# johndpope/SPEAK-hack

Hardware: NVIDIA B200
Metric: irfd_train_pairs_per_sec_256 (higher is better)
Workload: dtype bf16

## Files before the change

### speak_hack_b200/csrc/conv_gemm.cu

```cuda
#include <stdlib.h>

#include "host_util.h"
#include "ptx.cuh"

namespace irfd {

enum { EPI_PLAIN = 0, EPI_STATS = 1, EPI_STYLE = 2, EPI_AFFINE = 3, EPI_BNBWD = 4, EPI_BNBWD_RES = 5 };

struct ConvGemmArgs {
  int M_total, N_total;
  int num_m_tiles, num_n_tiles;
  int taps, kw, pad, cin_chunks;
  int H, W, HW, B;
  const float* bias;
  const float* nw;
  const float* noise;
  const float* sp1;
  const float* s1;
  float* stat_sum;
  float* stat_sq;
  const __nv_bfloat16* res;
  __nv_bfloat16* y_lo;
  int wg_tiles;
  int a_mod_tiles;
  int relu;
  const __nv_bfloat16* bn_z;
  const __nv_bfloat16* bn_g2;
  const uint8_t* bn_bits;
  const float* bn_mean;
  const float* bn_rstd;
  const float* bn_gamma[4];
  const float* bn_beta[4];
  int sg_tiles;
  int warp_epi;
};

constexpr int kNumThreads = 320;
constexpr int kEpiThreads = 256;
constexpr int kMiscBytes = 12 * 1024;
constexpr int kStgBytes = 16384;
constexpr int kSmemLimit = 232448;

template <int BLOCK_N, int MODE>
struct GemmCfg {
  static constexpr int A_BYTES = 128 * 128;
  static constexpr int B_BYTES = BLOCK_N * 128;
  static constexpr int STAGE_BYTES = A_BYTES + B_BYTES;
  static constexpr int NUM_OUT = (MODE == EPI_STYLE) ? 2 : 1;
  static constexpr int STG_TOTAL = 4 * kStgBytes;
  static constexpr int RAW_STAGES = (kSmemLimit - 1024 - STG_TOTAL - kMiscBytes) / STAGE_BYTES;
  static constexpr int STAGES = RAW_STAGES > 8 ? 8 : RAW_STAGES;
  static constexpr int SMEM_BYTES = 1024 + STAGES * STAGE_BYTES + STG_TOTAL + kMiscBytes;
  static constexpr uint32_t TMEM_COLS = (2 * BLOCK_N <= 128) ? 128 : (2 * BLOCK_N <= 256 ? 256 : 512);
};

template <int BLOCK_N, int MODE, int NBUF>
__device__ __forceinline__ void epilogue_acc(const ConvGemmArgs& p, const CUtensorMap* map_out,
                                             const CUtensorMap* map_out2, uint32_t tmem_base, uint32_t acc_col,
                                             int m0, int n_tile, uint64_t* release_bar, uint8_t* stg_base, float* vec,
                                             uint32_t& chunk_counter) {
  const int warp = threadIdx.x >> 5;
  const int lane = threadIdx.x & 31;
  const int e = warp - 2;
  const int q = warp & 3;
  const int half = e >> 2;
  const int etid = threadIdx.x - 64;
  const int r = q * 32 + lane;
  float* vb = vec;
  float* vnw = vec + 256;
  float* vsp1 = vec + 512;
  float* vs1 = vec + 1024;
  const int m_tile = m0 >> 7;
  const int ng0 = n_tile * BLOCK_N;
  const int pg0 = (m_tile / p.wg_tiles) * p.N_total + ng0;
  float noise_r = 0.f;
  int img_local = 0;
  if constexpr (MODE == EPI_STYLE) {
    const int nimg = p.HW < 128 ? 128 / p.HW : 1;
    const int b0 = m0 / p.HW;
    for (int i = etid; i < BLOCK_N; i += kEpiThreads) {
      vb[i] = p.bias[ng0 + i];
      vnw[i] = p.nw[ng0 + i];
    }
    for (int i = etid; i < nimg * BLOCK_N; i += kEpiThreads) {
      const int img = i / BLOCK_N, c = i - img * BLOCK_N;
      int bb = b0 + img;
      if (bb >= p.B) bb = p.B - 1;
      vsp1[img * 256 + c] = p.sp1[(size_t)bb * p.N_total + ng0 + c];
      vs1[img * 256 + c] = p.s1[(size_t)bb * p.N_total + ng0 + c];
    }
    named_bar_sync(1, kEpiThreads);
    if (m0 + r < p.M_total) noise_r = p.noise[m0 + r];
    img_local = p.HW < 128 ? r / p.HW : 0;
  } else if constexpr (MODE == EPI_PLAIN) {
    if (p.bias != nullptr) {
      for (int i = etid; i < BLOCK_N; i += kEpiThreads) vb[i] = p.bias[pg0 + i];
      named_bar_sync(1, kEpiThreads);
    }
  } else if constexpr (MODE == EPI_AFFINE) {
    for (int i = etid; i < BLOCK_N; i += kEpiThreads) {
      vb[i] = p.bias[pg0 + i];
      vnw[i] = p.nw[pg0 + i];
// ... 150 lines not shown
          tma_store_commit();
        }
      }
      if (etid < 128) {
        const int ch = etid & 63, which = etid >> 6;
        float acc = 0.f;
#pragma unroll
        for (int gg = 0; gg < 8; ++gg) acc += red[(gg * 64 + ch) * 2 + which];
        p.stat_sum[((size_t)m_tile * 2 + which) * p.N_total + ng0 + chunk * 64 + ch] = acc;
      }
      continue;
    }
    if (warp == 2) {
      __syncwarp();
      if (elect_one_sync()) {
        tma_store_2d(map_out, stg0, ng0 + chunk * 64, m0);
        if constexpr (MODE == EPI_STYLE) tma_store_2d(map_out2, stg1, ng0 + chunk * 64, m0);
        tma_store_commit();
      }
    }
    if constexpr (MODE == EPI_STATS) {
      const int pr = etid & 31;
      const int g = etid >> 5;
      float s0 = 0.f, s1 = 0.f, q0 = 0.f, q1 = 0.f;
#pragma unroll
      for (int i = 0; i < 16; ++i) {
        const int row = g * 16 + i;
        const int phys = (pr >> 2) ^ (row & 7);
        const uint32_t w = *reinterpret_cast<const uint32_t*>(stg0 + row * 128 + phys * 16 + (pr & 3) * 4);
        const float2 f = unpack_bf16x2(w);
        s0 += f.x;
        q0 += f.x * f.x;
        s1 += f.y;
        q1 += f.y * f.y;
      }
      float* red = vec;
      red[(g * 64 + 2 * pr) * 2 + 0] = s0;
      red[(g * 64 + 2 * pr) * 2 + 1] = q0;
      red[(g * 64 + 2 * pr + 1) * 2 + 0] = s1;
      red[(g * 64 + 2 * pr + 1) * 2 + 1] = q1;
      named_bar_sync(1, kEpiThreads);
      if (etid < 128) {
        const int ch = etid & 63, which = etid >> 6;
        float acc = 0.f;
#pragma unroll
        for (int gg = 0; gg < 8; ++gg) acc += red[(gg * 64 + ch) * 2 + which];
        float* dst = which ? p.stat_sq : p.stat_sum;
        dst[(size_t)m_tile * p.N_total + ng0 + chunk * 64 + ch] = acc;
      }
    }
  }
}

constexpr int kSlabBytes = 4096;

template <int BLOCK_N, int MODE>
__device__ __forceinline__ void epilogue_tile_warp(const ConvGemmArgs& p, const CUtensorMap* map_slab, uint32_t tmem_base,
                                                   uint32_t acc_col, int m0, int n_tile, uint64_t* release_bar,
                                                   uint8_t* stg_base, float* vec, uint32_t& chunk_counter,
                                                   uint32_t& my_slabs, bool release_at_leader = false) {
  static_assert(MODE != EPI_STYLE, "STYLE keeps the two-output epilogue");
  auto release = [&]() {
    if (release_at_leader) mbar_arrive_cluster(release_bar, 0);
    else mbar_arrive(release_bar);
  };
  constexpr int CHUNKS = BLOCK_N / 64;
  constexpr bool kSums = MODE == EPI_STATS || MODE == EPI_BNBWD || MODE == EPI_BNBWD_RES;
  const int warp = threadIdx.x >> 5;
  const int lane = threadIdx.x & 31;
  const int e = warp - 2;
  const int q = warp & 3;
  const int h = e >> 2;
  const int m_tile = m0 >> 7;
  const int ng0 = n_tile * BLOCK_N;
  const int pg0 = (m_tile / p.wg_tiles) * p.N_total + ng0;
  const int row = m0 + q * 32 + lane;
  uint8_t* slabs = stg_base + e * 2 * kSlabBytes;
  float* wvec = vec + e * 128;
  const int first = (h - (int)chunk_counter) & 1;
  const int last_mine = first < CHUNKS ? first + 2 * ((CHUNKS - 1 - first) / 2) : -1;
  if (last_mine < 0) {
    __syncwarp();
    if (lane == 0) release();
  }
#pragma unroll 1
  for (int chunk = first; chunk < CHUNKS; chunk += 2) {
    const int cg0 = ng0 + chunk * 64;
    uint32_t zw[32], gw[32];
    uint8_t bw[32];
    if constexpr (MODE == EPI_BNBWD || MODE == EPI_BNBWD_RES) {
      const size_t cell0 = (size_t)(m0 + q * 32) * p.N_total + cg0 + 2 * lane;
#pragma unroll
      for (int i = 0; i < 32; ++i) {
        zw[i] = __ldg(reinterpret_cast<const uint32_t*>(p.bn_z + cell0 + (size_t)i * p.N_total));
        if constexpr (MODE == EPI_BNBWD_RES) {
          gw[i] = __ldg(reinterpret_cast<const uint32_t*>(p.bn_g2 + cell0 + (size_t)i * p.N_total));
          bw[i] = __ldg(p.bn_bits + ((cell0 + (size_t)i * p.N_total) >> 3));
        }
      }
    }
    if constexpr (MODE == EPI_AFFINE || MODE == EPI_PLAIN) {
      if (MODE == EPI_AFFINE || p.bias != nullptr) {
        __syncwarp();
        wvec[lane] = MODE == EPI_AFFINE ? p.nw[pg0 + chunk * 64 + lane] : 0.f;
        wvec[lane + 32] = MODE == EPI_AFFINE ? p.nw[pg0 + chunk * 64 + 32 + lane] : 0.f;
        wvec[64 + lane] = p.bias[pg0 + chunk * 64 + lane];
        wvec[96 + lane] = p.bias[pg0 + chunk * 64 + 32 + lane];
        __syncwarp();
      }
    }
    uint32_t va[32], vb[32];
    const uint32_t taddr = tmem_base + (uint32_t(q * 32) << 16) + acc_col + chunk * 64;
    tmem_ld32(taddr, va);
    tmem_ld32(taddr + 32, vb);
    tmem_ld_wait();
    if (chunk == last_mine) {
      tc_fence_before();
      __syncwarp();
      if (lane == 0) release();
    }
    uint8_t* slab = slabs + (my_slabs & 1) * kSlabBytes;
    if (lane == 0) tma_store_wait_read<1>();
    __syncwarp();
#pragma unroll
    for (int j = 0; j < 8; ++j) {
      float o[8];
#pragma unroll
      for (int t = 0; t < 8; ++t) {
        const int c = j * 8 + t;
        const float acc = __uint_as_float(c < 32 ? va[c & 31] : vb[c & 31]);
        if constexpr (MODE == EPI_AFFINE) o[t] = acc * wvec[c] + wvec[64 + c];
        else if constexpr (MODE == EPI_PLAIN) o[t] = p.bias != nullptr ? acc + wvec[64 + c] : acc;
        else o[t] = acc;
      }
      if constexpr (MODE == EPI_AFFINE) {
        if (p.res != nullptr && row < p.M_total) {
          const uint4 u = *reinterpret_cast<const uint4*>(p.res + (size_t)row * p.N_total + cg0 + j * 8);
          const float2 a0 = unpack_bf16x2(u.x), a1 = unpack_bf16x2(u.y), a2 = unpack_bf16x2(u.z), a3 = unpack_bf16x2(u.w);
          o[0] += a0.x; o[1] += a0.y; o[2] += a1.x; o[3] += a1.y;
          o[4] += a2.x; o[5] += a2.y; o[6] += a3.x; o[7] += a3.y;
        }
#pragma unroll
        for (int t = 0; t < 8; ++t)
          o[t] = p.relu == 1 ? fmaxf(o[t], 0.f) : (p.relu == 2 ? (o[t] > 0.f ? o[t] : 0.2f * o[t]) : o[t]);
      }
      uint4 pk;
      pk.x = pack_bf16x2(o[0], o[1]);
      pk.y = pack_bf16x2(o[2], o[3]);
      pk.z = pack_bf16x2(o[4], o[5]);
      pk.w = pack_bf16x2(o[6], o[7]);
      *reinterpret_cast<uint4*>(slab + lane * 128 + ((j ^ (lane & 7)) << 4)) = pk;
    }
    if constexpr (kSums) {
      __syncwarp();
      float s0 = 0.f, s1 = 0.f, q0 = 0.f, q1 = 0.f;
      if constexpr (MODE == EPI_STATS) {
#pragma unroll
        for (int i = 0; i < 32; ++i) {
          const uint32_t w = *reinterpret_cast<const uint32_t*>(slab + i * 128 + (((lane >> 2) ^ (i & 7)) << 4) + (lane & 3) * 4);
          const float2 f = unpack_bf16x2(w);
          s0 += f.x;
          q0 += f.x * f.x;
          s1 += f.y;
          q1 += f.y * f.y;
        }
      } else {
        const int cc = cg0 + 2 * lane;
        const size_t so = (size_t)(m_tile / p.sg_tiles) * p.N_total + cc;
        const float2 mm = __ldg(reinterpret_cast<const float2*>(p.bn_mean + so));
        const float2 rs = __ldg(reinterpret_cast<const float2*>(p.bn_rstd + so));
        float2 ga = make_float2(0.f, 0.f), be = make_float2(0.f, 0.f);
        if constexpr (MODE == EPI_BNBWD) {
          const int grp = m_tile / p.wg_tiles;
          const float* gam =
              grp == 0 ? p.bn_gamma[0] : (grp == 1 ? p.bn_gamma[1] : (grp == 2 ? p.bn_gamma[2] : p.bn_gamma[3]));
          const float* bet = grp == 0 ? p.bn_beta[0] : (grp == 1 ? p.bn_beta[1] : (grp == 2 ? p.bn_beta[2] : p.bn_beta[3]));
          ga = __ldg(reinterpret_cast<const float2*>(gam + cc));
          be = __ldg(reinterpret_cast<const float2*>(bet + cc));
        }
        const int bit0 = (2 * lane) & 7;
#pragma unroll
        for (int i = 0; i < 32; ++i) {
          uint32_t* cell = reinterpret_cast<uint32_t*>(slab + i * 128 + (((lane >> 2) ^ (i & 7)) << 4) + (lane & 3) * 4);
          float2 f = unpack_bf16x2(*cell);
          const float2 z = unpack_bf16x2(zw[i]);
          const float x0 = (z.x - mm.x) * rs.x, x1 = (z.y - mm.y) * rs.y;
          if constexpr (MODE == EPI_BNBWD) {
            f.x = (ga.x * x0 + be.x) > 0.f ? f.x : 0.f;
            f.y = (ga.y * x1 + be.y) > 0.f ? f.y : 0.f;
          } else {
            const float2 g2 = unpack_bf16x2(gw[i]);
            f.x = ((bw[i] >> bit0) & 1) ? f.x + g2.x : 0.f;
            f.y = ((bw[i] >> (bit0 + 1)) & 1) ? f.y + g2.y : 0.f;
          }
          *cell = pack_bf16x2(f.x, f.y);
          s0 += f.x;
          q0 += f.x * x0;
          s1 += f.y;
          q1 += f.y * x1;
        }
      }
      float* red = vec + ((((my_slabs & 1) * 2 + h) * 4 + q) * 64) * 2;
      *reinterpret_cast<float4*>(red + 4 * lane) = make_float4(s0, q0, s1, q1);
    }
    fence_proxy_async_smem();
    __syncwarp();
    if (lane == 0) {
      tma_store_2d(map_slab, slab, cg0, m0 + q * 32);
      tma_store_commit();
    }
    if constexpr (kSums) {
      named_bar_sync(1 + h, 128);
      if (q == 0) {
        const float* r0 = vec + ((((my_slabs & 1) * 2 + h) * 4) * 64) * 2 + 4 * lane;
        float4 t = *reinterpret_cast<const float4*>(r0);
#pragma unroll
        for (int k = 1; k < 4; ++k) {
          const float4 u = *reinterpret_cast<const float4*>(r0 + k * 128);
          t.x += u.x;
          t.y += u.y;
          t.z += u.z;
          t.w += u.w;
        }
        if constexpr (MODE == EPI_STATS) {
          const size_t d = (size_t)m_tile * p.N_total + cg0 + 2 * lane;
          *reinterpret_cast<float2*>(p.stat_sum + d) = make_float2(t.x, t.z);
          *reinterpret_cast<float2*>(p.stat_sq + d) = make_float2(t.y, t.w);
        } else {
          const size_t d = (size_t)m_tile * 2 * p.N_total + cg0 + 2 * lane;
          *reinterpret_cast<float2*>(p.stat_sum + d) = make_float2(t.x, t.z);
          *reinterpret_cast<float2*>(p.stat_sum + d + p.N_total) = make_float2(t.y, t.w);
        }
      }
    }
    ++my_slabs;
  }
  chunk_counter += CHUNKS;
}

template <int BLOCK_N, int MODE, int CL = 1, bool MMA2 = false>
__global__ void __launch_bounds__(kNumThreads, 1)
conv_gemm_kernel(const __grid_constant__ CUtensorMap map_a, const __grid_constant__ CUtensorMap map_b,
                 const __grid_constant__ CUtensorMap map_out, const __grid_constant__ CUtensorMap map_out2,
                 const ConvGemmArgs p) {
  using Cfg = GemmCfg<BLOCK_N, MODE>;
  constexpr int STAGES = Cfg::STAGES;
  static_assert(STAGES >= 2, "pipeline too shallow");
  static_assert(!MMA2 || (CL == 2 && MODE != EPI_STYLE), "the 2-SM MMA needs a CTA pair and the per-warp epilogue");

  extern __shared__ uint8_t smem_raw[];
  uint8_t* smem = reinterpret_cast<uint8_t*>((reinterpret_cast<uintptr_t>(smem_raw) + 1023) & ~uintptr_t(1023));
  uint8_t* stg_base = smem + STAGES * Cfg::STAGE_BYTES;
  uint8_t* misc = stg_base + Cfg::STG_TOTAL;
  float* vec = reinterpret_cast<float*>(misc);
  uint64_t* full_bar = reinterpret_cast<uint64_t*>(misc + 8192);
  uint64_t* empty_bar = full_bar + STAGES;
  uint64_t* tmem_full = empty_bar + STAGES;
  uint64_t* tmem_empty = tmem_full + 2;
  uint32_t* tmem_ptr = reinterpret_cast<uint32_t*>(tmem_empty + 2);

  const int warp = threadIdx.x >> 5;
  const int lane = threadIdx.x & 31;
  const int crank = CL > 1 ? (int)cluster_ctarank() : 0;
  const int unit0 = blockIdx.x / CL, unit_step = gridDim.x / CL;
  const int total_units = (p.num_m_tiles / CL) * p.num_n_tiles;
  const int num_kb = p.taps * p.cin_chunks;
  constexpr uint16_t kClusterMask = (1u << CL) - 1;

  if (threadIdx.x == 0) {
    for (int i = 0; i < STAGES; ++i) {
      mbar_init(&full_bar[i], 1);
      mbar_init(&empty_bar[i], MMA2 ? 1 : CL);
    }
    for (int i = 0; i < 2; ++i) {
      mbar_init(&tmem_full[i], 1);
      mbar_init(&tmem_empty[i], MMA2 ? 16 : 8);
    }
    fence_mbar_init();
  }
  __syncwarp();
  if (warp == 0) {
    if (MMA2) tmem_alloc_2sm<Cfg::TMEM_COLS>(tmem_ptr);
    else tmem_alloc<Cfg::TMEM_COLS>(tmem_ptr);
  }
  tc_fence_before();
  __syncthreads();
  if (CL > 1) cluster_sync_all();
  tc_fence_after();
  const uint32_t tmem_base = *tmem_ptr;

  if (warp == 0) {
    {
      if (lane == 0) {
        tma_prefetch_desc(&map_a);
        tma_prefetch_desc(&map_b);
      }
      __syncwarp();
      int stage = 0;
      uint32_t phase = 0;
      for (int unit = unit0; unit < total_units; unit += unit_step) {
        const int m_tile = (unit / p.num_n_tiles) * CL + crank;
        const int n_tile = unit % p.num_n_tiles;
        const int m0 = (p.a_mod_tiles > 0 ? m_tile % p.a_mod_tiles : m_tile) * 128;
        const int w0 = m0 % p.W;
        const int h0 = (m0 / p.W) % p.H;
        const int n0 = m0 / (p.W * p.H);
        const int b_row = (m_tile / p.wg_tiles) * p.N_total + n_tile * BLOCK_N;
        for (int tap = 0; tap < p.taps; ++tap) {
          const int dh = tap / p.kw - p.pad;
          const int dw = tap % p.kw - p.pad;
          for (int ch = 0; ch < p.cin_chunks; ++ch) {
            mbar_wait(&empty_bar[stage], phase ^ 1);
            uint8_t* sa = smem + stage * Cfg::STAGE_BYTES;
            if (MMA2) {
              if (elect_one_sync()) {
                if (crank == 0) mbar_expect_tx(&full_bar[stage], 2 * (Cfg::A_BYTES + Cfg::B_BYTES / 2));
                tma_load_4d_2sm(sa, &map_a, &full_bar[stage], ch * 64, w0 + dw, h0 + dh, n0);
                tma_load_2d_2sm(sa + Cfg::A_BYTES, &map_b, &full_bar[stage], (tap * p.cin_chunks + ch) * 64,
                                b_row + crank * (BLOCK_N / 2));
              }
            } else if (elect_one_sync()) {
              mbar_expect_tx(&full_bar[stage], Cfg::STAGE_BYTES);
              tma_load_4d(sa, &map_a, &full_bar[stage], ch * 64, w0 + dw, h0 + dh, n0);
              if (CL == 1)
                tma_load_2d(sa + Cfg::A_BYTES, &map_b, &full_bar[stage], (tap * p.cin_chunks + ch) * 64, b_row);
              else
                tma_load_2d_mc(sa + Cfg::A_BYTES + crank * (Cfg::B_BYTES / CL), &map_b, &full_bar[stage],
                               (tap * p.cin_chunks + ch) * 64, b_row + crank * (BLOCK_N / CL), kClusterMask);
            }
            __syncwarp();
            if (++stage == STAGES) {
              stage = 0;
              phase ^= 1;
            }
          }
        }
      }
    }
  } else if (warp == 1) {
    if (!MMA2 || crank == 0) {
      constexpr uint32_t idesc = make_idesc_bf16(MMA2 ? 256 : 128, BLOCK_N, 0, 0);
      int stage = 0;
      uint32_t phase = 0;
      int iter = 0;
      for (int unit = unit0; unit < total_units; unit += unit_step, ++iter) {
        const int as = iter & 1;
        const uint32_t aphase = (iter >> 1) & 1;
        mbar_wait(&tmem_empty[as], aphase ^ 1);
        tc_fence_after();
        const uint32_t d_tmem = tmem_base + as * BLOCK_N;
        for (int kb = 0; kb < num_kb; ++kb) {
          mbar_wait(&full_bar[stage], phase);
          tc_fence_after();
          const uint32_t a_addr = smem_u32(smem + stage * Cfg::STAGE_BYTES);
          const uint64_t adesc0 = make_smem_desc_sw128(a_addr, 0, 1024);
          const uint64_t bdesc0 = make_smem_desc_sw128(a_addr + Cfg::A_BYTES, 0, 1024);
          if (elect_one_sync()) {
#pragma unroll
            for (int k = 0; k < 4; ++k)
              if (MMA2) umma_bf16_2sm(d_tmem, adesc0 + 2 * k, bdesc0 + 2 * k, idesc, (kb | k) != 0 ? 1u : 0u);
              else umma_bf16(d_tmem, adesc0 + 2 * k, bdesc0 + 2 * k, idesc, (kb | k) != 0 ? 1u : 0u);
            if (MMA2) umma_commit_2sm_mc(&empty_bar[stage], kClusterMask);
            else if (CL == 1) umma_commit(&empty_bar[stage]);
            else umma_commit_mc(&empty_bar[stage], kClusterMask);
          }
          __syncwarp();
          if (++stage == STAGES) {
            stage = 0;
            phase ^= 1;
          }
        }
        if (elect_one_sync()) {
          if (MMA2) umma_commit_2sm_mc(&tmem_full[as], kClusterMask);
          else umma_commit(&tmem_full[as]);
        }
        __syncwarp();
      }
    }
  } else {
    int iter = 0;
    uint32_t chunk_counter = 0, my_slabs = 0;
    for (int unit = unit0; unit < total_units; unit += unit_step, ++iter) {
      const int as = iter & 1;
      const uint32_t aphase = (iter >> 1) & 1;
      const int m_tile = (unit / p.num_n_tiles) * CL + crank;
      const int n_tile = unit % p.num_n_tiles;
      mbar_wait(&tmem_full[as], aphase);
      tc_fence_after();
      if constexpr (MODE != EPI_STYLE) {
        if (p.warp_epi) {
          epilogue_tile_warp<BLOCK_N, MODE>(p, &map_out2, tmem_base, as * BLOCK_N, m_tile * 128, n_tile, &tmem_empty[as],
                                            stg_base, vec, chunk_counter, my_slabs, MMA2);
          continue;
        }
      }
      epilogue_acc<BLOCK_N, MODE, 2>(p, &map_out, &map_out2, tmem_base, as * BLOCK_N, m_tile * 128, n_tile,
                                     &tmem_empty[as], stg_base, vec, chunk_counter);
    }
    if (MODE != EPI_STYLE && p.warp_epi) {
      if (lane == 0) tma_store_wait_read<0>();
    } else if (warp == 2) {
      __syncwarp();
      if (elect_one_sync()) tma_store_wait_read<0>();
    }
  }

  tc_fence_before();
  __syncthreads();
  if (CL > 1) cluster_sync_all();
  if (warp == 0) {
    if (MMA2) tmem_dealloc_2sm<Cfg::TMEM_COLS>(tmem_base);
    else tmem_dealloc<Cfg::TMEM_COLS>(tmem_base);
  }
}


constexpr int kHaloThreads = 352;
constexpr int kHaloCols = 130;
constexpr int kHaloRows = 4;

template <int BLOCK_N, int MODE>
struct HaloCfg {
  static_assert(BLOCK_N == 64 || BLOCK_N == 128, "two double-buffered accumulators need 4 x BLOCK_N <= 512 TMEM columns");
  static constexpr int A_BYTES = kHaloRows * kHaloCols * 128;
  static constexpr int A_STAGES = 2;
  static constexpr int B_BYTES = BLOCK_N * 128;
  static constexpr int NUM_OUT = (MODE == EPI_STYLE) ? 2 : 1;
  static constexpr int NBUF = (NUM_OUT == 2) ? 1 : 2;
  static constexpr int STG_TOTAL = NUM_OUT * NBUF * kStgBytes;
  static constexpr int RAW_B = (kSmemLimit - 1024 - A_STAGES * A_BYTES - STG_TOTAL - kMiscBytes) / B_BYTES;
  static constexpr int B_STAGES = RAW_B > 8 ? 8 : RAW_B;
  static constexpr int SMEM_BYTES = 1024 + A_STAGES * A_BYTES + B_STAGES * B_BYTES + STG_TOTAL + kMiscBytes;
  static constexpr uint32_t TMEM_COLS = 4 * BLOCK_N <= 256 ? 256 : 512;
  static_assert(A_BYTES % 1024 == 0 && B_STAGES >= 2, "halo stage must keep 1024-byte alignment");
};

struct HaloArgs {
  int wsegs, hpairs;
  int total_tiles;
};

template <int BLOCK_N, int MODE>
__global__ void __launch_bounds__(kHaloThreads, 1)
conv_halo_kernel(const __grid_constant__ CUtensorMap map_a, const __grid_constant__ CUtensorMap map_b,
                 const __grid_constant__ CUtensorMap map_out, const __grid_constant__ CUtensorMap map_out2,
// ... 291 lines not shown

struct BnBwdFold {
  const void* z;
  const float *mean, *rstd;
  const float* const* gamma;
  const float* const* beta;
  const void* g2;
  const void* bits;
  int stat_groups;
};

static int conv_gemm_impl(const void* x, int n, int h, int w, int cin, const void* wk, int cout, int ksize, void* out,
                          void* out2, void* out_lo, int mode, const float* bias, const float* nw, const float* noise,
                          const float* sp1, const float* s1, float* stat_sum, float* stat_sq, const void* res, int relu,
                          int force_block_n, cudaStream_t stream, int wgroups = 1, int a_shared = 0,
                          const BnBwdFold* fold = nullptr) {
  IRFD_CHECK_ARG(x && wk && out, "conv_gemm: null pointer");
  IRFD_CHECK_ARG(ksize == 1 || ksize == 3, "conv_gemm: ksize must be 1 or 3 (got %d)", ksize);
  IRFD_CHECK_ARG(cin % 64 == 0 && cin > 0, "conv_gemm: Cin must be a multiple of 64 (got %d)", cin);
  IRFD_CHECK_ARG(cout % 64 == 0 && cout > 0, "conv_gemm: Cout must be a multiple of 64 (got %d)", cout);
  IRFD_CHECK_ARG(mode >= 0 && mode <= 5, "conv_gemm: bad mode %d", mode);
  const long long m_total_ll = (long long)n * h * w;
  IRFD_CHECK_ARG(m_total_ll > 0 && m_total_ll < (1ll << 31) - 256, "conv_gemm: bad pixel count");
  const int m_total = (int)m_total_ll;
  IRFD_CHECK_ARG(wgroups == 1 || (wgroups > 1 && m_total_ll % (128ll * wgroups) == 0),
                 "conv_gemm: %d weight groups need a whole number of 128-pixel tiles per group (pixels %lld)", wgroups,
                 m_total_ll);
  IRFD_CHECK_ARG(wgroups == 1 || (mode != EPI_STYLE), "conv_gemm: weight groups are not available in STYLE mode");
  IRFD_CHECK_ARG(!a_shared || (ksize == 1 && wgroups > 1), "conv_gemm: a shared A operand needs ksize 1 and groups > 1");

  int H = h, W = w, NB = n;
  if (ksize == 1) {
    H = 1;
    W = a_shared ? m_total / wgroups : m_total;
    NB = 1;
  }
  int tw, th, tn;
  if (W >= 128) {
    IRFD_CHECK_ARG(ksize == 1 || W % 128 == 0, "conv_gemm: W=%d must be a multiple of 128", W);
    tw = 128; th = 1; tn = 1;
  } else {
    IRFD_CHECK_ARG(128 % W == 0, "conv_gemm: W=%d must divide 128", W);
    tw = W;
    const int rows = 128 / W;
    if (H >= rows) {
      IRFD_CHECK_ARG(H % rows == 0, "conv_gemm: H=%d must be a multiple of %d", H, rows);
      th = rows; tn = 1;
    } else {
      IRFD_CHECK_ARG(rows % H == 0, "conv_gemm: H=%d must divide %d", H, rows);
      th = H; tn = rows / H;
    }
  }

  ConvGemmArgs a;
  a.M_total = m_total;
  a.N_total = cout;
  a.num_m_tiles = (m_total + 127) / 128;
  a.taps = ksize * ksize;
  a.kw = ksize;
  a.pad = ksize / 2;
  a.cin_chunks = cin / 64;
  a.H = H; a.W = W; a.HW = h * w; a.B = n;
  a.bias = bias; a.nw = nw; a.noise = noise; a.sp1 = sp1; a.s1 = s1;
  a.stat_sum = stat_sum; a.stat_sq = stat_sq;
  a.res = reinterpret_cast<const __nv_bfloat16*>(res);
  a.y_lo = reinterpret_cast<__nv_bfloat16*>(out_lo);
  a.wg_tiles = wgroups > 1 ? a.num_m_tiles / wgroups : 0x7fffffff;
  a.a_mod_tiles = a_shared ? a.num_m_tiles / wgroups : 0;
  a.relu = relu;
  if (mode == EPI_AFFINE) IRFD_CHECK_ARG(bias && nw, "conv_gemm: AFFINE mode needs scale and shift");
  if (mode == EPI_STYLE) {
    IRFD_CHECK_ARG(bias && nw && noise && sp1 && s1 && out2, "conv_gemm: STYLE mode needs bias/nw/noise/sp1/s1/out2");
    IRFD_CHECK_ARG(h * w >= 64, "conv_gemm: STYLE mode needs >= 64 pixels per image");
  }
  if (mode == EPI_STATS) IRFD_CHECK_ARG(stat_sum && stat_sq, "conv_gemm: STATS mode needs stat buffers");
  a.warp_epi = (mode != EPI_STYLE && m_total % 128 == 0 && warp_epi_mode() != 0) ? 1 : 0;
  a.bn_z = nullptr;
  a.bn_mean = a.bn_rstd = nullptr;
  for (int i = 0; i < 4; ++i) a.bn_gamma[i] = a.bn_beta[i] = nullptr;
  a.sg_tiles = 0x7fffffff;
  a.bn_g2 = nullptr;
  a.bn_bits = nullptr;
  if (mode == EPI_BNBWD || mode == EPI_BNBWD_RES) {
    IRFD_CHECK_ARG(fold && fold->z && fold->mean && fold->rstd && stat_sum,
                   "conv_gemm: BNBWD modes need z, mean, rstd and the partial buffer");
    if (mode == EPI_BNBWD) IRFD_CHECK_ARG(fold->gamma && fold->beta, "conv_gemm: BNBWD mode needs gamma and beta");
    if (mode == EPI_BNBWD_RES)
      IRFD_CHECK_ARG(fold->g2 && fold->bits && cout % 8 == 0, "conv_gemm: BNBWD_RES mode needs g2 and the mask plane");
    IRFD_CHECK_ARG(wgroups <= 4 && m_total % 128 == 0 && fold->stat_groups >= wgroups &&
                       fold->stat_groups % wgroups == 0 && a.num_m_tiles % fold->stat_groups == 0,
                   "conv_gemm: BNBWD needs whole 128-pixel tiles per statistic group (%d tiles, %d groups, %d sets)",
                   a.num_m_tiles, fold->stat_groups, wgroups);
    a.bn_z = reinterpret_cast<const __nv_bfloat16*>(fold->z);
    a.bn_mean = fold->mean;
    a.bn_rstd = fold->rstd;
    for (int i = 0; i < wgroups && mode == EPI_BNBWD; ++i) {
      IRFD_CHECK_ARG(fold->gamma[i] && fold->beta[i], "conv_gemm: BNBWD gamma/beta pointer %d is null", i);
      a.bn_gamma[i] = fold->gamma[i];
      a.bn_beta[i] = fold->beta[i];
    }
    a.bn_g2 = reinterpret_cast<const __nv_bfloat16*>(fold->g2);
    a.bn_bits = reinterpret_cast<const uint8_t*>(fold->bits);
    a.sg_tiles = a.num_m_tiles / fold->stat_groups;
  }

  int block_n = force_block_n;
  if (block_n == 0) {
    block_n = 64;
    const int cands[3] = {256, 128, 64};
    for (int i = 0; i < 3; ++i) {
      if (cout % cands[i] == 0 && (long long)a.num_m_tiles * (cout / cands[i]) >= num_sms()) {
        block_n = cands[i];
        break;
      }
    }
    if (block_n == 64 && cout % 128 == 0 && (long long)a.num_m_tiles * (cout / 128) * 3 >= 2ll * num_sms()) block_n = 128;
  }
  IRFD_CHECK_ARG((block_n == 64 || block_n == 128 || block_n == 256) && cout % block_n == 0,
                 "conv_gemm: BLOCK_N %d incompatible with Cout %d", block_n, cout);
  const int hmode = halo_mode();
  const bool use_halo = hmode != 0 && mode != EPI_BNBWD && mode != EPI_BNBWD_RES && wgroups == 1 && ksize == 3 && W % 128 == 0 && H % 2 == 0 &&
                        (cout == 64 || cout == 128) &&
                        (force_block_n == 0 || force_block_n == cout);
  if (use_halo) block_n = cout;
  a.num_n_tiles = cout / block_n;
  int cluster = 1;
  if (!use_halo && (cluster_mode() != 0 || mma2_mode() != 0) && block_n >= 128 && a.num_m_tiles % 2 == 0 &&
      (wgroups == 1 || a.wg_tiles % 2 == 0) && (a.a_mod_tiles == 0 || a.a_mod_tiles % 2 == 0))
    cluster = (mma2_mode() != 0 && a.warp_epi && (mode == EPI_PLAIN || mode == EPI_STATS || mode == EPI_BNBWD)) ? 3 : 2;

  CUtensorMap ma, mb, mo, mo2;
  {
    const uint64_t dims[4] = {(uint64_t)cin, (uint64_t)W, (uint64_t)H, (uint64_t)NB};
    const uint64_t str[3] = {(uint64_t)cin * 2, (uint64_t)W * cin * 2, (uint64_t)H * W * cin * 2};
    uint32_t box[4] = {64, (uint32_t)tw, (uint32_t)th, (uint32_t)tn};
    if (use_halo) {
      box[1] = kHaloCols;
      box[2] = kHaloRows;
      box[3] = 1;
    }
    int rc = make_tmap_bf16(&ma, x, 4, dims, str, box, true);
    if (rc) return rc;
  }
  {
    const uint64_t ktot = (uint64_t)a.taps * cin;
    const uint64_t dims[2] = {ktot, (uint64_t)cout * wgroups};
    const uint64_t str[1] = {ktot * 2};
    const uint32_t box[2] = {64, (uint32_t)(block_n / (cluster > 1 ? 2 : 1))};
    int rc = make_tmap_bf16(&mb, wk, 2, dims, str, box, true);
    if (rc) return rc;
  }
  {
    const uint64_t dims[2] = {(uint64_t)cout, (uint64_t)m_total};
    const uint64_t str[1] = {(uint64_t)cout * 2};
    const uint32_t box[2] = {64, 128};
    int rc = make_tmap_bf16(&mo, out, 2, dims, str, box, true);
// ... 97 lines not shown
```

### speak_hack_b200/csrc/host_util.cu

```cuda
#include "host_util.h"

#include <mutex>
#include <unordered_set>

#include <stdarg.h>
#include <string.h>

namespace irfd {

static thread_local char g_last_error[512] = "";

void set_last_error(const char* fmt, ...) {
  va_list ap;
  va_start(ap, fmt);
  vsnprintf(g_last_error, sizeof(g_last_error), fmt, ap);
  va_end(ap);
}

EncodeTiledFn get_encode_tiled() {
  static EncodeTiledFn fn = nullptr;
  if (fn) return fn;
  void* p = nullptr;
  cudaDriverEntryPointQueryResult qres;
  cudaError_t e = cudaGetDriverEntryPoint("cuTensorMapEncodeTiled", &p, cudaEnableDefault, &qres);
  if (e != cudaSuccess || qres != cudaDriverEntryPointSuccess || p == nullptr) {
    set_last_error("cuTensorMapEncodeTiled entry point unavailable: %s", cudaGetErrorString(e));
    return nullptr;
  }
  fn = reinterpret_cast<EncodeTiledFn>(p);
  return fn;
}

int num_sms() {
  static int n = 0;
  if (n) return n;
  int dev = 0;
  cudaGetDevice(&dev);
  cudaDeviceGetAttribute(&n, cudaDevAttrMultiProcessorCount, dev);
  if (n <= 0) n = 148;
  return n;
}

int make_tmap_bf16(CUtensorMap* out, const void* base, int rank, const uint64_t* dims, const uint64_t* strides_bytes,
                   const uint32_t* box, bool swizzle128) {
  EncodeTiledFn enc = get_encode_tiled();
  if (!enc) return IRFD_ERR_CUDA;
  cuuint64_t gdims[5];
  cuuint64_t gstr[4];
  cuuint32_t gbox[5];
  cuuint32_t estr[5];
  for (int i = 0; i < rank; ++i) {
    gdims[i] = dims[i];
    gbox[i] = box[i];
    estr[i] = 1;
  }
  for (int i = 0; i + 1 < rank; ++i) gstr[i] = strides_bytes[i];
  CUresult r = enc(out, CU_TENSOR_MAP_DATA_TYPE_BFLOAT16, (cuuint32_t)rank, const_cast<void*>(base), gdims, gstr, gbox,
                   estr, CU_TENSOR_MAP_INTERLEAVE_NONE,
                   swizzle128 ? CU_TENSOR_MAP_SWIZZLE_128B : CU_TENSOR_MAP_SWIZZLE_NONE,
                   CU_TENSOR_MAP_L2_PROMOTION_L2_256B, CU_TENSOR_MAP_FLOAT_OOB_FILL_NONE);
  if (r != CUDA_SUCCESS) {
    set_last_error("cuTensorMapEncodeTiled failed (CUresult %d) rank=%d dims=[%llu,%llu,%llu,%llu] box=[%u,%u,%u,%u]",
                   (int)r, rank, (unsigned long long)dims[0], (unsigned long long)(rank > 1 ? dims[1] : 0),
                   (unsigned long long)(rank > 2 ? dims[2] : 0), (unsigned long long)(rank > 3 ? dims[3] : 0), box[0],
                   rank > 1 ? box[1] : 0, rank > 2 ? box[2] : 0, rank > 3 ? box[3] : 0);
    return IRFD_ERR_CUDA;
  }
  return IRFD_OK;
}

}

extern "C" const char* irfd_last_error(void) { return irfd::g_last_error; }

namespace irfd {
void prefer_max_shared_carveout(const void* kernel) {
  static std::mutex mu;
  static std::unordered_set<const void*> done;
  std::lock_guard<std::mutex> lock(mu);
  if (done.insert(kernel).second)
    cudaFuncSetAttribute(kernel, cudaFuncAttributePreferredSharedMemoryCarveout, cudaSharedmemCarveoutMaxShared);
}
}

extern "C" int irfd_abi_version(void) { return IRFD_ABI_VERSION; }
```

### speak_hack_b200/csrc/host_util.h

```cpp
#pragma once
#include <cuda.h>
#include <cuda_runtime.h>
#include <stdint.h>
#include <stdio.h>

#include "../../include/irfd_b200.h"

namespace irfd {

typedef CUresult (*EncodeTiledFn)(CUtensorMap*, CUtensorMapDataType, cuuint32_t, void*, const cuuint64_t*,
                                  const cuuint64_t*, const cuuint32_t*, const cuuint32_t*, CUtensorMapInterleave,
                                  CUtensorMapSwizzle, CUtensorMapL2promotion, CUtensorMapFloatOOBfill);

EncodeTiledFn get_encode_tiled();
int num_sms();
void set_last_error(const char* fmt, ...);

int make_tmap_bf16(CUtensorMap* out, const void* base, int rank, const uint64_t* dims, const uint64_t* strides_bytes,
                   const uint32_t* box, bool swizzle128);

void prefer_max_shared_carveout(const void* kernel);

#define IRFD_CHECK_ARG(cond, ...)            \
  do {                                       \
    if (!(cond)) {                           \
      irfd::set_last_error(__VA_ARGS__);     \
      return IRFD_ERR_INVALID_ARGUMENT;      \
    }                                        \
  } while (0)

#define IRFD_CHECK_LAUNCH()                                                        \
  do {                                                                             \
    cudaError_t e__ = cudaGetLastError();                                          \
    if (e__ != cudaSuccess) {                                                      \
      irfd::set_last_error("%s:%d CUDA launch: %s", __FILE__, __LINE__, cudaGetErrorString(e__)); \
      return IRFD_ERR_CUDA;                                                        \
    }                                                                              \
  } while (0)

}
```

### speak_hack_b200/encoder_group.py

```python
from __future__ import annotations

import os
from typing import Dict, List, Optional

import torch
import torch.nn as nn

from . import ops
from .encoder import BN_EPS, BN_MOMENTUM, ResNet50Encoder


fold_bn_reduce = os.environ.get("IRFD_BN_FOLD", "1") != "0"
fold_bn3_reduce = os.environ.get("IRFD_BN3_FOLD", "0") != "0"


def _stack_pack(convs, mode, kpad=0):
    return ops.pack_conv_weights_stacked([c.weight for c in convs], mode, kpad)


class _Stats:
    __slots__ = ("mean", "rstd")

    def __init__(self, mean, rstd):
        self.mean, self.rstd = mean, rstd


def _group_inference(grp: "EncoderGroup", x, col0=None):
    encs = grp.encoders
    E = len(encs)
    x = x.contiguous().to(torch.float32)
    n, _, h, w = x.shape
    if col0 is None:
        col0 = ops.im2col_stem(x, 192)
    sc, sh = ops.bn_eval_affine_sets([e[1] for e in encs])
    a0 = ops.conv_gemm_affine_grouped(col0, _stack_pack([e[0] for e in encs], ops.PACK_FLAT, 192), 1, sc, sh, relu=True,
                                      wgroups=E, a_shared=True).view(E * n, h // 2, w // 2, 64)
    cur, _ = ops.maxpool_fwd(a0)
    for li in range(4, 8):
        for bi in range(len(encs[0][li])):
            blks = [e[li][bi] for e in encs]
            nb, hh, ww, _cin = cur.shape
            sc, sh = ops.bn_eval_affine_sets([b.bn1 for b in blks])
            a1 = ops.conv_gemm_affine_grouped(cur, _stack_pack([b.conv1 for b in blks], ops.PACK_FPROP), 1, sc, sh,
                                              relu=True, wgroups=E)
            planes = a1.shape[-1]
            sc, sh = ops.bn_eval_affine_sets([b.bn2 for b in blks])
            wk2 = _stack_pack([b.conv2 for b in blks], ops.PACK_FPROP)
            if blks[0].stride == 1:
                a2 = ops.conv_gemm_affine_grouped(a1, wk2, 3, sc, sh, relu=True, wgroups=E)
            else:
                col2 = ops.im2col_3x3s2(a1)
                a2 = ops.conv_gemm_affine_grouped(col2.view(1, 1, col2.shape[0], 9 * planes), wk2, 1, sc, sh, relu=True,
                                                  wgroups=E).view(nb, hh // 2, ww // 2, planes)
            if blks[0].downsample is not None:
                xs = ops.subsample2(cur) if blks[0].stride == 2 else cur
                sc, sh = ops.bn_eval_affine_sets([b.downsample[1] for b in blks])
                idn = ops.conv_gemm_affine_grouped(xs, _stack_pack([b.downsample[0] for b in blks], ops.PACK_FPROP), 1,
                                                   sc, sh, relu=False, wgroups=E)
            else:
                idn = cur
            sc, sh = ops.bn_eval_affine_sets([b.bn3 for b in blks])
            cur = ops.conv_gemm_affine_grouped(a2, _stack_pack([b.conv3 for b in blks], ops.PACK_FPROP), 1, sc, sh,
                                               res=idn, relu=True, wgroups=E)
    return ops.avgpool_fwd(cur).view(E, n, -1, 1, 1)


# ... 228 lines not shown
```

Baseline: 902.2.

## Prefetch BN-backward side inputs via TMA into per-warp smem and enable BN3 fold

The BN-backward epilogue modes used to fetch z, g2 and the mask bits with per-lane strided __ldg loads into registers. They now issue TMA tile loads into per-warp shared-memory slots, one chunk ahead, gated by new mbarriers, and read the swizzled values from smem. The aim is to hide side-input latency, cut register pressure and get coalesced transfers. In exchange the staging area grows, which can reduce pipeline stages. BNBWD_RES now requires Cout to be a multiple of 128, and the BN3 fold path is enabled by default, which routes more layers through this epilogue.

```diff
diff --git a/speak_hack_b200/csrc/conv_gemm.cu b/speak_hack_b200/csrc/conv_gemm.cu
--- a/speak_hack_b200/csrc/conv_gemm.cu
+++ b/speak_hack_b200/csrc/conv_gemm.cu
@@ -8,6 +8,7 @@
 enum { EPI_PLAIN = 0, EPI_STATS = 1, EPI_STYLE = 2, EPI_AFFINE = 3, EPI_BNBWD = 4, EPI_BNBWD_RES = 5 };
 
 struct ConvGemmArgs {
+  CUtensorMap bn_z_map, bn_g2_map, bn_bits_map;
   int M_total, N_total;
   int num_m_tiles, num_n_tiles;
   int taps, kw, pad, cin_chunks;
@@ -41,13 +42,29 @@
 constexpr int kStgBytes = 16384;
 constexpr int kSmemLimit = 232448;
 
+constexpr int kSlabBytes = 4096;
+constexpr int kBitsBoxBytes = 512;
+
+constexpr int kNumSide = 1;
+constexpr int kSideBarOffset = 8192 + 256;
+constexpr int bn_side_bytes(int mode) {
+  return mode == EPI_BNBWD_RES ? 2 * kSlabBytes + kBitsBoxBytes : (mode == EPI_BNBWD ? kSlabBytes : 0);
+}
+constexpr int bn_warp_bytes(int mode, int nside) {
+  return (kSlabBytes + nside * bn_side_bytes(mode) + 1023) / 1024 * 1024;
+}
+
 template <int BLOCK_N, int MODE>
 struct GemmCfg {
   static constexpr int A_BYTES = 128 * 128;
   static constexpr int B_BYTES = BLOCK_N * 128;
   static constexpr int STAGE_BYTES = A_BYTES + B_BYTES;
   static constexpr int NUM_OUT = (MODE == EPI_STYLE) ? 2 : 1;
-  static constexpr int STG_TOTAL = 4 * kStgBytes;
+  static constexpr bool BN_SIDE = MODE == EPI_BNBWD || MODE == EPI_BNBWD_RES;
+  static constexpr int NSIDE = BN_SIDE ? kNumSide : 0;
+  static constexpr int WARP_BYTES = BN_SIDE ? bn_warp_bytes(MODE, NSIDE) : 2 * kSlabBytes;
+  static constexpr int STG_TOTAL = BN_SIDE ? 8 * WARP_BYTES : 4 * kStgBytes;
+  static_assert(STG_TOTAL >= 2 * kStgBytes, "epilogue_acc needs two staging tiles");
   static constexpr int RAW_STAGES = (kSmemLimit - 1024 - STG_TOTAL - kMiscBytes) / STAGE_BYTES;
   static constexpr int STAGES = RAW_STAGES > 8 ? 8 : RAW_STAGES;
   static constexpr int SMEM_BYTES = 1024 + STAGES * STAGE_BYTES + STG_TOTAL + kMiscBytes;
@@ -304,14 +321,42 @@
   }
 }
 
-constexpr int kSlabBytes = 4096;
-
-template <int BLOCK_N, int MODE>
+
+template <int BLOCK_N, int MODE, int CL>
+__device__ __forceinline__ void bn_side_load(const ConvGemmArgs& p, uint8_t* region, uint64_t* side_bar, uint32_t k) {
+  using Cfg = GemmCfg<BLOCK_N, MODE>;
+  constexpr int CHUNKS = BLOCK_N / 64;
+  const int warp = threadIdx.x >> 5;
+  const int q = warp & 3, h = (warp - 2) >> 2;
+  const uint32_t g = (uint32_t)h + 2 * k;
+  const int unit = (int)(blockIdx.x / CL) + (int)(g / CHUNKS) * (int)(gridDim.x / CL);
+  if (unit >= (p.num_m_tiles / CL) * p.num_n_tiles) return;
+  const int m_tile = (unit / p.num_n_tiles) * CL + (CL > 1 ? (int)cluster_ctarank() : 0);
+  const int cg0 = (unit % p.num_n_tiles) * BLOCK_N + (int)(g % CHUNKS) * 64;
+  const int row0 = m_tile * 128 + q * 32;
+  const int s = (int)(k % Cfg::NSIDE);
+  uint64_t* bar = side_bar + s;
+  uint8_t* zs = region + kSlabBytes + s * kSlabBytes;
+  if constexpr (MODE == EPI_BNBWD_RES) {
+    mbar_expect_tx(bar, 2 * kSlabBytes + kBitsBoxBytes);
+    tma_load_2d(zs, &p.bn_z_map, bar, cg0, row0);
+    tma_load_2d(zs + Cfg::NSIDE * kSlabBytes, &p.bn_g2_map, bar, cg0, row0);
+    tma_load_2d(region + kSlabBytes + 2 * Cfg::NSIDE * kSlabBytes + s * kBitsBoxBytes, &p.bn_bits_map, bar,
+                (cg0 >> 7) << 4, row0);
+  } else {
+    mbar_expect_tx(bar, kSlabBytes);
+    tma_load_2d(zs, &p.bn_z_map, bar, cg0, row0);
+  }
+}
+
+template <int BLOCK_N, int MODE, int CL>
 __device__ __forceinline__ void epilogue_tile_warp(const ConvGemmArgs& p, const CUtensorMap* map_slab, uint32_t tmem_base,
                                                    uint32_t acc_col, int m0, int n_tile, uint64_t* release_bar,
                                                    uint8_t* stg_base, float* vec, uint32_t& chunk_counter,
                                                    uint32_t& my_slabs, bool release_at_leader = false) {
   static_assert(MODE != EPI_STYLE, "STYLE keeps the two-output epilogue");
+  using Cfg = GemmCfg<BLOCK_N, MODE>;
+  constexpr bool kSide = Cfg::BN_SIDE;
   auto release = [&]() {
     if (release_at_leader) mbar_arrive_cluster(release_bar, 0);
     else mbar_arrive(release_bar);
@@ -327,7 +372,8 @@
   const int ng0 = n_tile * BLOCK_N;
   const int pg0 = (m_tile / p.wg_tiles) * p.N_total + ng0;
   const int row = m0 + q * 32 + lane;
-  uint8_t* slabs = stg_base + e * 2 * kSlabBytes;
+  uint64_t* side_bar = reinterpret_cast<uint64_t*>(reinterpret_cast<uint8_t*>(vec) + kSideBarOffset) + e * Cfg::NSIDE;
+  uint8_t* slabs = stg_base + e * Cfg::WARP_BYTES;
   float* wvec = vec + e * 128;
   const int first = (h - (int)chunk_counter) & 1;
   const int last_mine = first < CHUNKS ? first + 2 * ((CHUNKS - 1 - first) / 2) : -1;
@@ -338,19 +384,6 @@
 #pragma unroll 1
   for (int chunk = first; chunk < CHUNKS; chunk += 2) {
     const int cg0 = ng0 + chunk * 64;
-    uint32_t zw[32], gw[32];
-    uint8_t bw[32];
-    if constexpr (MODE == EPI_BNBWD || MODE == EPI_BNBWD_RES) {
-      const size_t cell0 = (size_t)(m0 + q * 32) * p.N_total + cg0 + 2 * lane;
-#pragma unroll
-      for (int i = 0; i < 32; ++i) {
-        zw[i] = __ldg(reinterpret_cast<const uint32_t*>(p.bn_z + cell0 + (size_t)i * p.N_total));
-        if constexpr (MODE == EPI_BNBWD_RES) {
-          gw[i] = __ldg(reinterpret_cast<const uint32_t*>(p.bn_g2 + cell0 + (size_t)i * p.N_total));
-          bw[i] = __ldg(p.bn_bits + ((cell0 + (size_t)i * p.N_total) >> 3));
-        }
-      }
-    }
     if constexpr (MODE == EPI_AFFINE || MODE == EPI_PLAIN) {
       if (MODE == EPI_AFFINE || p.bias != nullptr) {
         __syncwarp();
@@ -371,8 +404,11 @@
       __syncwarp();
       if (lane == 0) release();
     }
-    uint8_t* slab = slabs + (my_slabs & 1) * kSlabBytes;
-    if (lane == 0) tma_store_wait_read<1>();
+    uint8_t* slab = kSide ? slabs : slabs + (my_slabs & 1) * kSlabBytes;
+    if (lane == 0) {
+      if constexpr (kSide) tma_store_wait_read<0>();
+      else tma_store_wait_read<1>();
+    }
     __syncwarp();
 #pragma unroll
     for (int j = 0; j < 8; ++j) {
@@ -431,19 +467,27 @@
           be = __ldg(reinterpret_cast<const float2*>(bet + cc));
         }
         const int bit0 = (2 * lane) & 7;
+        const int s = (int)(my_slabs % Cfg::NSIDE);
+        const uint8_t* zs = slabs + kSlabBytes + s * kSlabBytes;
+        const uint8_t* gs = zs + Cfg::NSIDE * kSlabBytes;
+        const uint8_t* bs = slabs + kSlabBytes + 2 * Cfg::NSIDE * kSlabBytes + s * kBitsBoxBytes + ((cg0 >> 6) & 1) * 8 +
+                            (lane >> 2);
+        mbar_wait(side_bar + s, (my_slabs / Cfg::NSIDE) & 1);
 #pragma unroll
         for (int i = 0; i < 32; ++i) {
-          uint32_t* cell = reinterpret_cast<uint32_t*>(slab + i * 128 + (((lane >> 2) ^ (i & 7)) << 4) + (lane & 3) * 4);
+          const int off = i * 128 + (((lane >> 2) ^ (i & 7)) << 4) + (lane & 3) * 4;
+          uint32_t* cell = reinterpret_cast<uint32_t*>(slab + off);
           float2 f = unpack_bf16x2(*cell);
-          const float2 z = unpack_bf16x2(zw[i]);
+          const float2 z = unpack_bf16x2(*reinterpret_cast<const uint32_t*>(zs + off));
           const float x0 = (z.x - mm.x) * rs.x, x1 = (z.y - mm.y) * rs.y;
           if constexpr (MODE == EPI_BNBWD) {
             f.x = (ga.x * x0 + be.x) > 0.f ? f.x : 0.f;
             f.y = (ga.y * x1 + be.y) > 0.f ? f.y : 0.f;
           } else {
-            const float2 g2 = unpack_bf16x2(gw[i]);
-            f.x = ((bw[i] >> bit0) & 1) ? f.x + g2.x : 0.f;
-            f.y = ((bw[i] >> (bit0 + 1)) & 1) ? f.y + g2.y : 0.f;
+            const float2 g2 = unpack_bf16x2(*reinterpret_cast<const uint32_t*>(gs + off));
+            const uint32_t bw = bs[i * 16];
+            f.x = ((bw >> bit0) & 1) ? f.x + g2.x : 0.f;
+            f.y = ((bw >> (bit0 + 1)) & 1) ? f.y + g2.y : 0.f;
           }
           *cell = pack_bf16x2(f.x, f.y);
           s0 += f.x;
@@ -460,6 +504,7 @@
     if (lane == 0) {
       tma_store_2d(map_slab, slab, cg0, m0 + q * 32);
       tma_store_commit();
+      if constexpr (kSide) bn_side_load<BLOCK_N, MODE, CL>(p, slabs, side_bar, my_slabs + Cfg::NSIDE);
     }
     if constexpr (kSums) {
       named_bar_sync(1 + h, 128);
@@ -494,14 +539,14 @@
 __global__ void __launch_bounds__(kNumThreads, 1)
 conv_gemm_kernel(const __grid_constant__ CUtensorMap map_a, const __grid_constant__ CUtensorMap map_b,
                  const __grid_constant__ CUtensorMap map_out, const __grid_constant__ CUtensorMap map_out2,
-                 const ConvGemmArgs p) {
+                 const __grid_constant__ ConvGemmArgs p) {
   using Cfg = GemmCfg<BLOCK_N, MODE>;
   constexpr int STAGES = Cfg::STAGES;
   static_assert(STAGES >= 2, "pipeline too shallow");
   static_assert(!MMA2 || (CL == 2 && MODE != EPI_STYLE), "the 2-SM MMA needs a CTA pair and the per-warp epilogue");
 
   extern __shared__ uint8_t smem_raw[];
-  uint8_t* smem = reinterpret_cast<uint8_t*>((reinterpret_cast<uintptr_t>(smem_raw) + 1023) & ~uintptr_t(1023));
+  uint8_t* smem = smem_raw + ((1024u - (smem_u32(smem_raw) & 1023u)) & 1023u);
   uint8_t* stg_base = smem + STAGES * Cfg::STAGE_BYTES;
   uint8_t* misc = stg_base + Cfg::STG_TOTAL;
   float* vec = reinterpret_cast<float*>(misc);
@@ -510,6 +555,8 @@
   uint64_t* tmem_full = empty_bar + STAGES;
   uint64_t* tmem_empty = tmem_full + 2;
   uint32_t* tmem_ptr = reinterpret_cast<uint32_t*>(tmem_empty + 2);
+  uint64_t* side_bar = reinterpret_cast<uint64_t*>(misc + kSideBarOffset);
+  static_assert(16 * STAGES + 32 + 4 <= 256, "barrier area");
 
   const int warp = threadIdx.x >> 5;
   const int lane = threadIdx.x & 31;
@@ -528,6 +575,7 @@
       mbar_init(&tmem_full[i], 1);
       mbar_init(&tmem_empty[i], MMA2 ? 16 : 8);
     }
+    for (int i = 0; i < 8 * Cfg::NSIDE; ++i) mbar_init(&side_bar[i], 1);
     fence_mbar_init();
   }
   __syncwarp();
@@ -632,6 +680,20 @@
   } else {
     int iter = 0;
     uint32_t chunk_counter = 0, my_slabs = 0;
+    if constexpr (Cfg::BN_SIDE) {
+      if (p.warp_epi && lane == 0) {
+        if (warp == 2) {
+          tma_prefetch_desc(&p.bn_z_map);
+          if (MODE == EPI_BNBWD_RES) {
+            tma_prefetch_desc(&p.bn_g2_map);
+            tma_prefetch_desc(&p.bn_bits_map);
+          }
+        }
+        for (int k = 0; k < Cfg::NSIDE; ++k)
+          bn_side_load<BLOCK_N, MODE, CL>(p, stg_base + (warp - 2) * Cfg::WARP_BYTES,
+                                          side_bar + (warp - 2) * Cfg::NSIDE, k);
+      }
+    }
     for (int unit = unit0; unit < total_units; unit += unit_step, ++iter) {
       const int as = iter & 1;
       const uint32_t aphase = (iter >> 1) & 1;
@@ -641,8 +703,8 @@
       tc_fence_after();
       if constexpr (MODE != EPI_STYLE) {
         if (p.warp_epi) {
-          epilogue_tile_warp<BLOCK_N, MODE>(p, &map_out2, tmem_base, as * BLOCK_N, m_tile * 128, n_tile, &tmem_empty[as],
-                                            stg_base, vec, chunk_counter, my_slabs, MMA2);
+          epilogue_tile_warp<BLOCK_N, MODE, CL>(p, &map_out2, tmem_base, as * BLOCK_N, m_tile * 128, n_tile,
+                                                &tmem_empty[as], stg_base, vec, chunk_counter, my_slabs, MMA2);
           continue;
         }
       }
@@ -1040,7 +1102,7 @@
     }
   }
 
-  ConvGemmArgs a;
+  ConvGemmArgs a{};
   a.M_total = m_total;
   a.N_total = cout;
   a.num_m_tiles = (m_total + 127) / 128;
@@ -1074,7 +1136,8 @@
                    "conv_gemm: BNBWD modes need z, mean, rstd and the partial buffer");
     if (mode == EPI_BNBWD) IRFD_CHECK_ARG(fold->gamma && fold->beta, "conv_gemm: BNBWD mode needs gamma and beta");
     if (mode == EPI_BNBWD_RES)
-      IRFD_CHECK_ARG(fold->g2 && fold->bits && cout % 8 == 0, "conv_gemm: BNBWD_RES mode needs g2 and the mask plane");
+      IRFD_CHECK_ARG(fold->g2 && fold->bits && cout % 128 == 0,
+                     "conv_gemm: BNBWD_RES mode needs g2, the mask plane and Cout %% 128 == 0 (got %d)", cout);
     IRFD_CHECK_ARG(wgroups <= 4 && m_total % 128 == 0 && fold->stat_groups >= wgroups &&
                        fold->stat_groups % wgroups == 0 && a.num_m_tiles % fold->stat_groups == 0,
                    "conv_gemm: BNBWD needs whole 128-pixel tiles per statistic group (%d tiles, %d groups, %d sets)",
@@ -1090,6 +1153,20 @@
     a.bn_g2 = reinterpret_cast<const __nv_bfloat16*>(fold->g2);
     a.bn_bits = reinterpret_cast<const uint8_t*>(fold->bits);
     a.sg_tiles = a.num_m_tiles / fold->stat_groups;
+    const uint64_t dims[2] = {(uint64_t)cout, (uint64_t)m_total};
+    const uint64_t str[1] = {(uint64_t)cout * 2};
+    const uint32_t box[2] = {64, 32};
+    int rc = make_tmap_bf16(&a.bn_z_map, fold->z, 2, dims, str, box, true);
+    if (rc) return rc;
+    if (mode == EPI_BNBWD_RES) {
+      rc = make_tmap_bf16(&a.bn_g2_map, fold->g2, 2, dims, str, box, true);
+      if (rc) return rc;
+      const uint64_t bdims[2] = {(uint64_t)cout / 8, (uint64_t)m_total};
+      const uint64_t bstr[1] = {(uint64_t)cout / 8};
+      const uint32_t bbox[2] = {16, 32};
+      rc = make_tmap_u8(&a.bn_bits_map, fold->bits, 2, bdims, bstr, bbox);
+      if (rc) return rc;
+    }
   }
 
   int block_n = force_block_n;
diff --git a/speak_hack_b200/csrc/host_util.cu b/speak_hack_b200/csrc/host_util.cu
--- a/speak_hack_b200/csrc/host_util.cu
+++ b/speak_hack_b200/csrc/host_util.cu
@@ -41,8 +41,8 @@
   return n;
 }
 
-int make_tmap_bf16(CUtensorMap* out, const void* base, int rank, const uint64_t* dims, const uint64_t* strides_bytes,
-                   const uint32_t* box, bool swizzle128) {
+static int make_tmap(CUtensorMap* out, CUtensorMapDataType dtype, const void* base, int rank, const uint64_t* dims,
+                     const uint64_t* strides_bytes, const uint32_t* box, bool swizzle128) {
   EncodeTiledFn enc = get_encode_tiled();
   if (!enc) return IRFD_ERR_CUDA;
   cuuint64_t gdims[5];
@@ -55,7 +55,7 @@
     estr[i] = 1;
   }
   for (int i = 0; i + 1 < rank; ++i) gstr[i] = strides_bytes[i];
-  CUresult r = enc(out, CU_TENSOR_MAP_DATA_TYPE_BFLOAT16, (cuuint32_t)rank, const_cast<void*>(base), gdims, gstr, gbox,
+  CUresult r = enc(out, dtype, (cuuint32_t)rank, const_cast<void*>(base), gdims, gstr, gbox,
                    estr, CU_TENSOR_MAP_INTERLEAVE_NONE,
                    swizzle128 ? CU_TENSOR_MAP_SWIZZLE_128B : CU_TENSOR_MAP_SWIZZLE_NONE,
                    CU_TENSOR_MAP_L2_PROMOTION_L2_256B, CU_TENSOR_MAP_FLOAT_OOB_FILL_NONE);
@@ -67,6 +67,16 @@
     return IRFD_ERR_CUDA;
   }
   return IRFD_OK;
+}
+
+int make_tmap_bf16(CUtensorMap* out, const void* base, int rank, const uint64_t* dims, const uint64_t* strides_bytes,
+                   const uint32_t* box, bool swizzle128) {
+  return make_tmap(out, CU_TENSOR_MAP_DATA_TYPE_BFLOAT16, base, rank, dims, strides_bytes, box, swizzle128);
+}
+
+int make_tmap_u8(CUtensorMap* out, const void* base, int rank, const uint64_t* dims, const uint64_t* strides_bytes,
+                 const uint32_t* box) {
+  return make_tmap(out, CU_TENSOR_MAP_DATA_TYPE_UINT8, base, rank, dims, strides_bytes, box, false);
 }
 
 }
diff --git a/speak_hack_b200/csrc/host_util.h b/speak_hack_b200/csrc/host_util.h
--- a/speak_hack_b200/csrc/host_util.h
+++ b/speak_hack_b200/csrc/host_util.h
@@ -18,6 +18,8 @@
 
 int make_tmap_bf16(CUtensorMap* out, const void* base, int rank, const uint64_t* dims, const uint64_t* strides_bytes,
                    const uint32_t* box, bool swizzle128);
+int make_tmap_u8(CUtensorMap* out, const void* base, int rank, const uint64_t* dims, const uint64_t* strides_bytes,
+                 const uint32_t* box);
 
 void prefer_max_shared_carveout(const void* kernel);
 
diff --git a/speak_hack_b200/encoder_group.py b/speak_hack_b200/encoder_group.py
--- a/speak_hack_b200/encoder_group.py
+++ b/speak_hack_b200/encoder_group.py
@@ -11,7 +11,7 @@
 
 
 fold_bn_reduce = os.environ.get("IRFD_BN_FOLD", "1") != "0"
-fold_bn3_reduce = os.environ.get("IRFD_BN3_FOLD", "0") != "0"
+fold_bn3_reduce = os.environ.get("IRFD_BN3_FOLD", "1") != "0"
 
 
 def _stack_pack(convs, mode, kpad=0):
```

Measured after the change: 920.3 (median of 6 runs). 1.02x the previous value.
